# gaspachoo/EEG2Video

Measured on AMD Instinct MI355X. Metric: 6-frame 288x512 clips/sec (50-step DDIM), higher is better.
Workload: dtype f32; 1 GPU; 1xMI355X: batch=8/GPU synthetic latents [B,4,6,36,64] + [B,77,768] cond, 50-step DDIM, CFG 12.5, 288x512x6 VAE decode, fp32 (BASELINE configs[1]); clips_per_gpu=8, ddim_steps=50, unet_samples_per_ddim_step=16, weights=random-init SD-v1-4 architecture, counter RNG seed 42/43, collective=none

## Files before the change

eeg2video_amd/csrc/attn.hip:

```cpp
#include "h16.h"
#include "kernels.h"
#include "prof.h"
#include "runtime.h"
#include "act_io.h"

#include <cstdlib>
#include <type_traits>

namespace e2v {

typedef float f32x16 __attribute__((ext_vector_type(16)));
typedef float f32x4 __attribute__((ext_vector_type(4)));

struct AttnBlock { int qb, head, sf; bool valid; };
__host__ __device__ __forceinline__ int attn_xcd_unit(const int n, const int F, const int heads) {
    return n % 8 == 0 ? 0 : (n * F) % 8 == 0 ? 1 : 2;
}
__device__ __forceinline__ AttnBlock attn_block_of(const AttnArgs& p, const int nqb) {
    const int b = blockIdx.x, xcd = b & 7, idx = b >> 3;
    const int S = p.n * p.F;
    const int unit = attn_xcd_unit(p.n, p.F, p.heads);
    AttnBlock r;
    if (unit == 0) {
        const int per = p.F * p.heads * nqb;
        const int ul = idx / per, w = idx - ul * per;
        const int smp = ul * 8 + xcd;
        const int f = w / (p.heads * nqb), w2 = w - f * (p.heads * nqb);
        r.sf = smp * p.F + f; r.head = w2 / nqb; r.qb = w2 - r.head * nqb; r.valid = smp < p.n;
    } else if (unit == 1) {
        const int per = p.heads * nqb;
        const int ul = idx / per, w = idx - ul * per;
        r.sf = ul * 8 + xcd; r.head = w / nqb; r.qb = w - r.head * nqb; r.valid = r.sf < S;
    } else {
        const int ul = idx / nqb;
        const int pair = ul * 8 + xcd;
        r.qb = idx - ul * nqb; r.sf = pair / p.heads; r.head = pair - r.sf * p.heads; r.valid = pair < S * p.heads;
    }
    return r;
}
__device__ __forceinline__ AttnBlock attn_block(const AttnArgs& p) { return attn_block_of(p, (p.Nq + 127) / 128); }
static inline unsigned attn_grid_of(const AttnArgs& a, const unsigned nqb) {
    const int unit = attn_xcd_unit(a.n, a.F, a.heads);
    if (unit == 0) return 8u * (a.n / 8) * (unsigned)(a.F * a.heads) * nqb;
    if (unit == 1) return 8u * ((a.n * a.F) / 8) * (unsigned)a.heads * nqb;
    return 8u * ((a.n * a.F * a.heads + 7) / 8) * nqb;
}
static inline unsigned attn_grid(const AttnArgs& a) { return attn_grid_of(a, (a.Nq + 127) / 128); }

std::string attn_shape_tag(const AttnArgs& a) {
    return " D" + std::to_string(a.D) + " Nq" + std::to_string(a.Nq) + " Nk" + std::to_string(a.Nk) + " n" + std::to_string(a.n) + " F" + std::to_string(a.F) +
           " h" + std::to_string(a.heads);
}

template <int D>
__global__ __launch_bounds__(256) void flash_attn_kernel(const AttnArgs p) {
    constexpr int LD = D + 4;
    constexpr int TF = D / 32;
    constexpr bool VREM = (D - 32 * TF) == 8;
    constexpr int T = VREM ? TF : (D + 31) / 32;
    constexpr int TA = T > 0 ? T : 1;
    constexpr int G = D / 8;
    constexpr int DQ = D / 4;
    constexpr int KT = 32;
    constexpr int NF4 = KT * DQ;
    constexpr int LPT = (NF4 + 255) / 256;
    extern __shared__ __attribute__((aligned(16))) float smem[];

    const int tid = threadIdx.x;
    const int lane = tid & 63, wave = tid >> 6;
    const int j = lane & 31, h = lane >> 5;
    const AttnBlock blk = attn_block(p);
    if (!blk.valid) return;
    const int sf = blk.sf;
    const int smp = sf / p.F, f = sf - smp * p.F;
    const int head = blk.head;
    const int q0 = (blk.qb * 4 + wave) * 32;
    const bool active = q0 < p.Nq;

    int nseg = 1;
    size_t kvbase[2];
    if (p.mode == 0) {
        kvbase[0] = (size_t)(smp * p.F) * p.Nk;
        kvbase[1] = (size_t)(smp * p.F + (f > 0 ? f - 1 : 0)) * p.Nk;
        nseg = f >= 2 ? 2 : 1;
    } else {
        kvbase[0] = kvbase[1] = (size_t)smp * p.Nk;
    }
    const int tps = (p.Nk + KT - 1) / KT;
    const int ntiles = nseg * tps;

    f32x4 qf[G];
    {
        const int qrow = min(q0 + j, p.Nq - 1);
        const float* qp = p.q + ((size_t)sf * p.Nq + qrow) * p.ldq + head * D + h * 4;
        const float c = p.scale * 1.44269504088896340736f;
#pragma unroll
        for (int g = 0; g < G; ++g) {
            qf[g] = *reinterpret_cast<const f32x4*>(qp + g * 8);
            qf[g] *= c;
        }
    }

    constexpr unsigned OOB = 0x80000000u;
    auto rsrc_of = [](const void* ptr) {
        const unsigned long long v = reinterpret_cast<unsigned long long>(ptr);
        const unsigned lo = __builtin_amdgcn_readfirstlane((unsigned)v);
        const unsigned hi = __builtin_amdgcn_readfirstlane((unsigned)(v >> 32));
        return __builtin_amdgcn_make_buffer_rsrc(reinterpret_cast<void*>(((unsigned long long)hi << 32) | lo), (short)0, 0x7FFFFFF0,
                                                 0x00020000);
    };
    int ld_row[LPT];
    unsigned ld_off[LPT];
#pragma unroll
    for (int e = 0; e < LPT; ++e) {
        const int idx = tid + 256 * e;
        const int row = idx / DQ, c4 = idx - row * DQ;
        ld_row[e] = row;
        ld_off[e] = idx < NF4 ? (unsigned)(row * p.ldkv + c4 * 4) * 4u : OOB;
    }
    f32x4 kreg[LPT], vreg[LPT];
    auto load_tile = [&](int tt) {
        const int seg = tt / tps;
        const int key0 = (tt - seg * tps) * KT;
        const size_t first = (kvbase[seg] + key0) * p.ldkv + head * D;
        const __amdgpu_buffer_rsrc_t rk = rsrc_of(p.k + first), rv = rsrc_of(p.v + first);
        const int left = p.Nk - key0;
#pragma unroll
        for (int e = 0; e < LPT; ++e) {
            unsigned off = ld_off[e];
            if (left < KT) off = ld_row[e] < left ? off : OOB;
            kreg[e] = __builtin_bit_cast(f32x4, __builtin_amdgcn_raw_buffer_load_b128(rk, off, 0, 0));
            vreg[e] = __builtin_bit_cast(f32x4, __builtin_amdgcn_raw_buffer_load_b128(rv, off, 0, 0));
        }
    };
    auto store_tile = [&](int buf) {
        float* Ks = smem + buf * (2 * KT * LD);
        float* Vs = Ks + KT * LD;
#pragma unroll
        for (int e = 0; e < LPT; ++e) {
            const int idx = tid + 256 * e;
            if (idx < NF4) {
                const int row = idx / DQ, c4 = idx - row * DQ;
                *reinterpret_cast<f32x4*>(Ks + row * LD + c4 * 4) = kreg[e];
                *reinterpret_cast<f32x4*>(Vs + row * LD + c4 * 4) = vreg[e];
            }
        }
    };

    f32x16 acc[TA];
#pragma unroll
    for (int t = 0; t < TA; ++t)
#pragma unroll
        for (int r = 0; r < 16; ++r) acc[t][r] = 0.f;
    f32x4 rem0 = {0.f, 0.f, 0.f, 0.f}, rem1 = {0.f, 0.f, 0.f, 0.f};
    float m_i = -INFINITY, l_i = 0.f;

    load_tile(0);
    store_tile(0);
    __syncthreads();

    for (int tt = 0; tt < ntiles; ++tt) {
        const int buf = tt & 1;
        if (tt + 1 < ntiles) load_tile(tt + 1);
        const int seg_c = tt / tps;
        const int kbase = (tt - seg_c * tps) * KT;
        auto tile_body = [&](const int key0, const int sub, auto ragged) {
            const float* Ks = smem + buf * (2 * KT * LD) + sub * 32 * LD;
            const float* Vs = smem + buf * (2 * KT * LD) + KT * LD + sub * 32 * LD;
            const f32x16 zero16 = {0.f, 0.f, 0.f, 0.f, 0.f, 0.f, 0.f, 0.f, 0.f, 0.f, 0.f, 0.f, 0.f, 0.f, 0.f, 0.f};
            f32x16 st;
            const float* kp = Ks + j * LD + h * 4;
#pragma unroll
            for (int g = 0; g < G; ++g) {
                const f32x4 kf = *reinterpret_cast<const f32x4*>(kp + g * 8);
#pragma unroll
                for (int s = 0; s < 4; ++s)
                    st = __builtin_amdgcn_mfma_f32_32x32x2f32(kf[s], qf[g][s], (g == 0 && s == 0) ? zero16 : st, 0, 0, 0);
            }
            if constexpr (decltype(ragged)::value) {
#pragma unroll
                for (int r = 0; r < 16; ++r) {
                    const int key = key0 + (r & 3) + 8 * (r >> 2) + 4 * h;
                    if (key >= p.Nk) st[r] = -INFINITY;
                }
            }
            float mt = st[0];
#pragma unroll
            for (int r = 1; r < 16; ++r) mt = __builtin_fmaxf(mt, st[r]);
            mt = __builtin_fmaxf(mt, __shfl_xor(mt, 32));
            const float m_new = __builtin_fmaxf(m_i, mt);
            const bool moved = __any(m_new > m_i);
            float ps = 0.f;
#pragma unroll
            for (int r = 0; r < 16; ++r) {
                st[r] = __builtin_amdgcn_exp2f(st[r] - m_new);
                ps += st[r];
            }
            float alpha = 1.0f;
            if (moved) {
                alpha = __builtin_amdgcn_exp2f(m_i - m_new);
                l_i *= alpha;
            }
            l_i += ps;
            m_i = m_new;
#pragma unroll
            for (int t = 0; t < T; ++t) {
                if (moved) {
#pragma unroll
                    for (int r = 0; r < 16; ++r) acc[t][r] *= alpha;
                }
                const int dv = min(t * 32 + j, D - 1);
                const float* vp = Vs + (4 * h) * LD + dv;
#pragma unroll
                for (int r = 0; r < 16; ++r) {
                    const float vv = vp[((r & 3) + 8 * (r >> 2)) * LD];
                    acc[t] = __builtin_amdgcn_mfma_f32_32x32x2f32(vv, st[r], acc[t], 0, 0, 0);
                }
            }
            if constexpr (VREM) {
                if (moved) {
                    rem0 *= alpha;
                    rem1 *= alpha;
                }
                const float* vr = Vs + (4 * h) * LD + 32 * TF;
#pragma unroll
                for (int r = 0; r < 16; ++r) {
                    const float* row = vr + ((r & 3) + 8 * (r >> 2)) * LD;
                    const f32x4 v0 = *reinterpret_cast<const f32x4*>(row);
                    const f32x4 v1 = *reinterpret_cast<const f32x4*>(row + 4);
                    rem0 += v0 * st[r];
                    rem1 += v1 * st[r];
                }
            }
        };
#pragma unroll
        for (int sub = 0; sub < KT / 32; ++sub) {
            const int key0 = kbase + 32 * sub;
            if (active && key0 < p.Nk) {
                if (key0 + 32 <= p.Nk) tile_body(key0, sub, std::false_type{});
                else tile_body(key0, sub, std::true_type{});
            }
        }
        if (tt + 1 < ntiles) store_tile(buf ^ 1);
        __syncthreads();
    }

    const float l_tot = l_i + __shfl_xor(l_i, 32);
    if constexpr (VREM) {
#pragma unroll
        for (int e = 0; e < 4; ++e) {
            rem0[e] += __shfl_xor(rem0[e], 32);
            rem1[e] += __shfl_xor(rem1[e], 32);
        }
    }
    if (active && q0 + j < p.Nq) {
        const float inv = 1.0f / l_tot;
        float* op = p.o + ((size_t)sf * p.Nq + q0 + j) * p.ldo + head * D;
#pragma unroll
        for (int t = 0; t < T; ++t)
#pragma unroll
            for (int rg = 0; rg < 4; ++rg) {
                const int dv = t * 32 + 8 * rg + 4 * h;
                if (dv < D) {
                    f32x4 o;
#pragma unroll
                    for (int e = 0; e < 4; ++e) o[e] = acc[t][rg * 4 + e] * inv;
                    *reinterpret_cast<f32x4*>(op + dv) = o;
                }
            }
        if constexpr (VREM) {
            const f32x4 o = (h ? rem1 : rem0) * inv;
            *reinterpret_cast<f32x4*>(op + 32 * TF + 4 * h) = o;
        }
    }
}

typedef __bf16 abf16x4 __attribute__((ext_vector_type(4)));
typedef __bf16 abf16x8 __attribute__((ext_vector_type(8)));

template <typename H, int D, bool FOLD, int KT>
__global__ __launch_bounds__(256) void flash_attn_b16io_kernel(const AttnArgs p) {
    constexpr int DP = (D + 15) / 16 * 16;
    constexpr int KS = DP / 16;
    constexpr int T = (D + 31) / 32;
    constexpr int KROW = DP * 2 + 16;
    constexpr int VROW = ((T * 16) % 32 == 16) ? T * 64 : T * 64 + 64;
    constexpr int KBYTES = KT * KROW, VBYTES = KT * VROW;
    constexpr int STAGE = (KBYTES + VBYTES + 15) / 16 * 16;
    constexpr bool SUMV = (D % 32) != 0;
    constexpr int LROW = D % 32, LREG = 4 * (LROW / 8) + (LROW & 3), LHALF = (LROW >> 2) & 1;
    constexpr int C8 = D / 8;
    constexpr int NP = KT * C8;
    constexpr int LPT = (NP + 255) / 256;
    extern __shared__ __attribute__((aligned(16))) char smem_h[];

    const int tid = threadIdx.x;
    const int lane = tid & 63, wave = tid >> 6;
    const int j = lane & 31, h = lane >> 5;
    const AttnBlock blk = attn_block(p);
    if (!blk.valid) return;
    const int sf = blk.sf;
    const int smp = sf / p.F, f = sf - smp * p.F;
    const int head = blk.head;
    const int q0 = (blk.qb * 4 + wave) * 32;
    const bool active = q0 < p.Nq;
    const H* __restrict__ Q = reinterpret_cast<const H*>(p.q);
    const H* __restrict__ K = reinterpret_cast<const H*>(p.k);
    const H* __restrict__ V = reinterpret_cast<const H*>(p.v);

    int nseg = 1;
    size_t kvbase[2];
    if (p.mode == 0) {
        kvbase[0] = (size_t)(smp * p.F) * p.Nk;
        kvbase[1] = (size_t)(smp * p.F + (f > 0 ? f - 1 : 0)) * p.Nk;
        nseg = f >= 2 ? 2 : 1;
    } else {
        kvbase[0] = kvbase[1] = (size_t)smp * p.Nk;
    }
    const int tps = (p.Nk + KT - 1) / KT;
    const int ntiles = nseg * tps;

    for (int i = tid * 16; i < 2 * STAGE; i += 256 * 16)
        *reinterpret_cast<f32x4*>(smem_h + i) = f32x4{0.f, 0.f, 0.f, 0.f};
    if constexpr (SUMV) {
        __syncthreads();
        if (tid < 2 * KT)
            *reinterpret_cast<H*>(smem_h + (tid / KT) * STAGE + KBYTES + (tid % KT) * VROW + D * 2) = (H)1.0f;
    }

    hx8<H> qf[KS];
    {
        const int qrow = min(q0 + j, p.Nq - 1);
        const H* qp = Q + ((size_t)sf * p.Nq + qrow) * p.ldq + head * D;
#pragma unroll
        for (int s = 0; s < KS; ++s) {
            const int k0 = 16 * s + 8 * h;
            hx8<H> a;
#pragma unroll
            for (int e = 0; e < 8; ++e) a[e] = (H)0.f;
            if (k0 < D) a = *reinterpret_cast<const hx8<H>*>(qp + k0);
            if constexpr (FOLD) {
                const float qs = p.scale * 1.44269504088896340736f;
#pragma unroll
                for (int e = 0; e < 8; ++e) a[e] = (H)((float)a[e] * qs);
            }
            qf[s] = a;
        }
    }
    const float sc = p.scale * 1.44269504088896340736f;
    __syncthreads();

    constexpr unsigned OOB = 0x80000000u;
    auto rsrc_of = [](const void* ptr) {
        const unsigned long long v = reinterpret_cast<unsigned long long>(ptr);
        const unsigned lo = __builtin_amdgcn_readfirstlane((unsigned)v);
        const unsigned hi = __builtin_amdgcn_readfirstlane((unsigned)(v >> 32));
        return __builtin_amdgcn_make_buffer_rsrc(reinterpret_cast<void*>(((unsigned long long)hi << 32) | lo), (short)0, 0x7FFFFFF0,
                                                 0x00020000);
    };
    int ld_row[LPT], ld_c8[LPT];
    unsigned ld_off[LPT];
#pragma unroll
    for (int e = 0; e < LPT; ++e) {
        const int idx = tid + 256 * e;
        const int row = idx / C8, c8 = idx - row * C8;
        ld_row[e] = row; ld_c8[e] = c8;
        ld_off[e] = idx < NP ? (unsigned)(row * p.ldkv + c8 * 8) * 2u : OOB;
    }
    f32x4 kreg[LPT], vreg[LPT];
    auto load_tile = [&](const int seg, const int key0) {
        const size_t first = (kvbase[seg] + key0) * p.ldkv + head * D;
        const __amdgpu_buffer_rsrc_t rk = rsrc_of(K + first), rv = rsrc_of(V + first);
        const int left = p.Nk - key0;
#pragma unroll
        for (int e = 0; e < LPT; ++e) {
            unsigned off = ld_off[e];
            if (left < KT) off = ld_row[e] < left ? off : OOB;
            kreg[e] = __builtin_bit_cast(f32x4, __builtin_amdgcn_raw_buffer_load_b128(rk, off, 0, 0));
            vreg[e] = __builtin_bit_cast(f32x4, __builtin_amdgcn_raw_buffer_load_b128(rv, off, 0, 0));
        }
    };
    auto store_tile = [&](int buf) {
        char* Kl = smem_h + buf * STAGE;
        char* Vl = Kl + KBYTES;
#pragma unroll
        for (int e = 0; e < LPT; ++e) {
            if (tid + 256 * e < NP) {
                *reinterpret_cast<f32x4*>(Kl + ld_row[e] * KROW + ld_c8[e] * 16) = kreg[e];
                *reinterpret_cast<f32x4*>(Vl + ld_row[e] * VROW + ld_c8[e] * 16) = vreg[e];
            }
        }
    };

    f32x16 acc[T];
#pragma unroll
    for (int t = 0; t < T; ++t)
#pragma unroll
        for (int r = 0; r < 16; ++r) acc[t][r] = 0.f;
    float m_i = -INFINITY, l_i = 0.f;
    f32x16 negm;
#pragma unroll
    for (int r = 0; r < 16; ++r) negm[r] = 0.f;

    load_tile(0, 0);
    store_tile(0);
    __syncthreads();

    const int ti = lane & 15;
    const int tr_off = (4 * h + (ti >> 2)) * VROW + (16 * ((lane >> 4) & 1) + 4 * (ti & 3)) * 2;

    int key0 = 0;
    for (int tt = 0; tt < ntiles; ++tt) {
        const int buf = tt & 1;
        if (tt == tps) key0 = 0;
        if (tt + 1 < ntiles) {
            if (tt + 1 == tps) load_tile(1, 0); else load_tile(tt + 1 > tps ? 1 : 0, key0 + KT);
        }
#pragma unroll
        for (int sub = 0; sub < KT / 32; ++sub) {
        const int keyb = key0 + 32 * sub;
        if (active && keyb < p.Nk) {
            const char* Kl = smem_h + buf * STAGE + sub * 32 * KROW;
            const char* Vl = smem_h + buf * STAGE + KBYTES + sub * 32 * VROW;
            const f32x16 zero16 = {0.f, 0.f, 0.f, 0.f, 0.f, 0.f, 0.f, 0.f, 0.f, 0.f, 0.f, 0.f, 0.f, 0.f, 0.f, 0.f};
            f32x16 st;
            const char* kp = Kl + j * KROW + h * 16;
#pragma unroll
            for (int s = 0; s < KS; ++s) {
// ... 465 lines not shown
                for (int x = 0; x < 4; ++x) {
                    unsigned v1, v2, v3;
                    split3(vreg[e][x], v1, v2, v3);
                    char* vd = Vl + (c4 * 4 + x) * VROW + row * 2;
                    *reinterpret_cast<unsigned short*>(vd) = (unsigned short)(v1 >> 16);
                    *reinterpret_cast<unsigned short*>(vd + VBYTES) = (unsigned short)(v2 >> 16);
                    *reinterpret_cast<unsigned short*>(vd + 2 * VBYTES) = (unsigned short)(v3 >> 16);
                }
            }
        }
    };

    f32x16 acc[T];
#pragma unroll
    for (int t = 0; t < T; ++t)
#pragma unroll
        for (int r = 0; r < 16; ++r) acc[t][r] = 0.f;
    float m_i = -INFINITY, l_i = 0.f;

    load_tile(0);
    store_tile(0);
    __syncthreads();

    constexpr int TA[6] = {1, 2, 0, 1, 0, 0}, TB[6] = {1, 0, 2, 0, 1, 0};
    for (int tt = 0; tt < ntiles; ++tt) {
        const int buf = tt & 1;
        if (tt + 1 < ntiles) load_tile(tt + 1);
        const int seg_c = tt / tps;
        const int key0 = (tt - seg_c * tps) * 32;
        if (active) {
            const char* Kl = smem_x + buf * STAGE;
            const char* Vl = Kl + 3 * KBYTES;
            f32x16 st;
#pragma unroll
            for (int r = 0; r < 16; ++r) st[r] = 0.f;
            const char* kp = Kl + j * KROW + h * 16;
#pragma unroll
            for (int s = 0; s < KS; ++s) {
                abf16x8 kf[3];
#pragma unroll
                for (int pl = 0; pl < 3; ++pl) kf[pl] = *reinterpret_cast<const abf16x8*>(kp + pl * KBYTES + s * 32);
#pragma unroll
                for (int t6 = 0; t6 < 6; ++t6)
                    st = __builtin_amdgcn_mfma_f32_32x32x16_bf16(kf[TA[t6]], __builtin_bit_cast(abf16x8, qf[TB[t6]][s]), st, 0, 0, 0);
            }
            if (key0 + 32 > p.Nk) {
#pragma unroll
                for (int r = 0; r < 16; ++r) {
                    const int key = key0 + (r & 3) + 8 * (r >> 2) + 4 * h;
                    if (key >= p.Nk) st[r] = -INFINITY;
                }
            }
            float mt = st[0];
#pragma unroll
            for (int r = 1; r < 16; ++r) mt = __builtin_fmaxf(mt, st[r]);
            mt = __builtin_fmaxf(mt, __shfl_xor(mt, 32));
            const float m_new = __builtin_fmaxf(m_i, mt);
            const bool moved = __any(m_new > m_i);
            float ps = 0.f;
#pragma unroll
            for (int r = 0; r < 16; ++r) {
                st[r] = __builtin_amdgcn_exp2f(st[r] - m_new);
                ps += st[r];
            }
            float alpha = 1.0f;
            if (moved) {
                alpha = __builtin_amdgcn_exp2f(m_i - m_new);
                l_i *= alpha;
            }
            l_i += ps;
            m_i = m_new;
            au32x4 pf[3][2];
#pragma unroll
            for (int s = 0; s < 2; ++s)
#pragma unroll
                for (int e = 0; e < 4; ++e) {
                    unsigned a1, a2, a3, b1, b2, b3;
                    split3(st[8 * s + 2 * e], a1, a2, a3);
                    split3(st[8 * s + 2 * e + 1], b1, b2, b3);
                    pf[0][s][e] = (a1 >> 16) | (b1 & 0xFFFF0000u);
                    pf[1][s][e] = (a2 >> 16) | (b2 & 0xFFFF0000u);
                    pf[2][s][e] = (a3 >> 16) | (b3 & 0xFFFF0000u);
                }
#pragma unroll
            for (int t = 0; t < T; ++t) {
                if (moved) {
#pragma unroll
                    for (int r = 0; r < 16; ++r) acc[t][r] *= alpha;
                }
                const char* vrow = Vl + min(t * 32 + j, D - 1) * VROW + h * 8;
#pragma unroll
                for (int s = 0; s < 2; ++s) {
                    abf16x8 vf[3];
#pragma unroll
                    for (int pl = 0; pl < 3; ++pl) {
                        const abf16x4 lo = *reinterpret_cast<const abf16x4*>(vrow + pl * VBYTES + s * 32);
                        const abf16x4 hi = *reinterpret_cast<const abf16x4*>(vrow + pl * VBYTES + s * 32 + 16);
                        vf[pl] = __builtin_shufflevector(lo, hi, 0, 1, 2, 3, 4, 5, 6, 7);
                    }
#pragma unroll
                    for (int t6 = 0; t6 < 6; ++t6)
                        acc[t] = __builtin_amdgcn_mfma_f32_32x32x16_bf16(vf[TA[t6]], __builtin_bit_cast(abf16x8, pf[TB[t6]][s]), acc[t], 0, 0, 0);
                }
            }
        }
        if (tt + 1 < ntiles) store_tile(buf ^ 1);
        __syncthreads();
    }

    const float l_tot = l_i + __shfl_xor(l_i, 32);
    if (active && q0 + j < p.Nq) {
        const float inv = 1.0f / l_tot;
        float* op = p.o + ((size_t)sf * p.Nq + q0 + j) * p.ldo + head * D;
#pragma unroll
        for (int t = 0; t < T; ++t)
#pragma unroll
            for (int rg = 0; rg < 4; ++rg) {
                const int dv = t * 32 + 8 * rg + 4 * h;
                if (dv < D) {
                    f32x4 o;
#pragma unroll
                    for (int e = 0; e < 4; ++e) o[e] = acc[t][rg * 4 + e] * inv;
                    *reinterpret_cast<f32x4*>(op + dv) = o;
                }
            }
    }
}
template <int D>
static void launch_flash_x3(const AttnArgs& a, hipStream_t s) {
    constexpr int DP = (D + 15) / 16 * 16;
    constexpr size_t stage = ((size_t)3 * (32 * (DP * 2 + 16) + ((D + 31) / 32) * 32 * 72) + 15) / 16 * 16;
    constexpr size_t smem = 2 * stage;
    E2V_KATTR(&flash_attn_x3_kernel<D>, smem);
    dim3 grid(attn_grid(a), 1, 1);
    const double nk = a.mode == 0 ? 2.0 * a.Nk : (double)a.Nk;
    const double probs = (double)a.n * a.F * a.heads;
    ProfScope ps(a.mode == 0 ? "flash_attn_f32x3_sparse_causal" : "flash_attn_f32x3_cross", 4.0 * probs * a.Nq * nk * D,
                 4.0 * probs * D * (2.0 * a.Nq + 2.0 * (a.mode == 0 ? a.Nk : (double)a.Nk / a.F)), s);
    E2V_KLAUNCH((flash_attn_x3_kernel<D>), grid, dim3(256), smem, s, a);
}

template <int D>
static void launch_flash(const AttnArgs& a, hipStream_t s) {
    constexpr size_t smem = (size_t)2 * 2 * 32 * (D + 4) * sizeof(float);
    E2V_KATTR(&flash_attn_kernel<D>, smem);
    dim3 grid(attn_grid(a), 1, 1);
    const double nk = a.mode == 0 ? 2.0 * a.Nk : (double)a.Nk;
    const double probs = (double)a.n * a.F * a.heads;
    std::string pname = a.mode == 0 ? "flash_attn_sparse_causal" : "flash_attn_cross";
    if (prof_detail()) pname += attn_shape_tag(a);
    ProfScope ps(pname.c_str(), 4.0 * probs * a.Nq * nk * D,
                 4.0 * probs * D * (2.0 * a.Nq + 2.0 * (a.mode == 0 ? a.Nk : (double)a.Nk / a.F)), s);
    dry_tag(" -> flash_attn_kernel");
    E2V_KLAUNCH((flash_attn_kernel<D>), grid, dim3(256), smem, s, a);
}

bool flash_attention_supports(int D) {
    switch (D) {
        case 8: case 16: case 32: case 40: case 64: case 80: case 160: return true;
        default: return false;
    }
}

void flash_attention(const AttnArgs& a, hipStream_t s) {
    if (!flash_attention_supports(a.D))
        throw Error(E2V_EINVAL, "attention head dim " + std::to_string(a.D) + " has no kernel instance (supported: 8, 16, 32, 40, 64, 80, 160)");
    if (a.io_bf16) {
        if ((a.ldq | a.ldkv | a.ldo) & 7) throw Error(E2V_ESHAPE, "bf16 attention: row strides must be multiples of 8 elements");
        switch (a.D) {
            case 8: launch_flash_b16io<8>(a, s); return;
            case 16: launch_flash_b16io<16>(a, s); return;
            case 32: launch_flash_b16io<32>(a, s); return;
            case 40: launch_flash_b16io<40>(a, s); return;
            case 64: launch_flash_b16io<64>(a, s); return;
            case 80: launch_flash_b16io<80>(a, s); return;
            default: launch_flash_b16io<160>(a, s); return;
        }
    }
    if (a.x3) {
        switch (a.D) {
            case 8: launch_flash_x3<8>(a, s); return;
            case 16: launch_flash_x3<16>(a, s); return;
            case 32: launch_flash_x3<32>(a, s); return;
            case 40: launch_flash_x3<40>(a, s); return;
            case 64: launch_flash_x3<64>(a, s); return;
            case 80: launch_flash_x3<80>(a, s); return;
            default: launch_flash_x3<160>(a, s); return;
        }
    }
    switch (a.D) {
        case 8: launch_flash<8>(a, s); break;
        case 16: launch_flash<16>(a, s); break;
        case 32: launch_flash<32>(a, s); break;
        case 40: launch_flash<40>(a, s); break;
        case 64: launch_flash<64>(a, s); break;
        case 80: launch_flash<80>(a, s); break;
        default: launch_flash<160>(a, s); break;
    }
}

static constexpr int FMAX = 8;
template <typename T>
__global__ __launch_bounds__(256) void temporal_attn_kernel(const T* __restrict__ qkv, int ld, T* __restrict__ out,
                                                            int ldo, int n, int F, int HW, int heads, int D, float scale) {
    const size_t total = (size_t)n * HW * heads * F;
    const size_t gid = blockIdx.x * (size_t)blockDim.x + threadIdx.x;
    if (gid >= total) return;
    const int i = gid % F;
    const int head = (gid / F) % heads;
    const size_t ph = gid / ((size_t)F * heads);
    const int pix = ph % HW;
    const int smp = ph / HW;
    const int C = heads * D;
    const size_t row0 = (size_t)smp * F * HW + pix;
    const T* qp = qkv + (row0 + (size_t)i * HW) * ld + head * D;
    const T* kp = qkv + row0 * ld + C + head * D;
    const T* vp = qkv + row0 * ld + 2 * C + head * D;
    const size_t fstride = (size_t)HW * ld;
    float s[FMAX];
#pragma unroll
    for (int jf = 0; jf < FMAX; ++jf) s[jf] = 0.f;
    for (int c = 0; c < D; c += 4) {
        const f32x4 qv = ld4(qp + c);
#pragma unroll
        for (int jf = 0; jf < FMAX; ++jf)
            if (jf < F) {
                const f32x4 kv = ld4(kp + jf * fstride + c);
                s[jf] += qv[0] * kv[0] + qv[1] * kv[1] + qv[2] * kv[2] + qv[3] * kv[3];
            }
    }
    float m = -INFINITY;
#pragma unroll
    for (int jf = 0; jf < FMAX; ++jf)
        if (jf < F) {
            s[jf] *= scale;
            m = fmaxf(m, s[jf]);
        }
    float l = 0.f;
#pragma unroll
    for (int jf = 0; jf < FMAX; ++jf)
        if (jf < F) {
            s[jf] = expf(s[jf] - m);
            l += s[jf];
        }
    const float inv = 1.0f / l;
    T* op = out + (row0 + (size_t)i * HW) * ldo + head * D;
    for (int c = 0; c < D; c += 4) {
        f32x4 o = {0.f, 0.f, 0.f, 0.f};
#pragma unroll
        for (int jf = 0; jf < FMAX; ++jf)
            if (jf < F) {
                const f32x4 vv = ld4(vp + jf * fstride + c);
                o += vv * (s[jf] * inv);
            }
        st4(op + c, o);
    }
}

template <typename T>
__global__ __launch_bounds__(128) void temporal_attn_lds_kernel(const T* __restrict__ qkv, int ld, T* __restrict__ out,
                                                                int ldo, int F, int HW, int C, int D, float scale, int PB,
                                                                int CS, int npg) {
    extern __shared__ __attribute__((aligned(16))) float sm[];
    const int smp = blockIdx.x / npg, p0 = (blockIdx.x - smp * npg) * PB;
    const int c_base = blockIdx.y * CS;
    if constexpr (!std::is_same<T, float>::value) {
        const int CO = CS / 8;
        const int total = F * PB * 3 * CO;
        for (int idx = threadIdx.x; idx < total; idx += 128) {
            const int c8 = idx % CO;
            int r = idx / CO;
            const int part = r % 3; r /= 3;
            const int pp = r % PB;
            const int f = r / PB;
            const int pix = p0 + pp;
            f32x4 lo = {0.f, 0.f, 0.f, 0.f}, hi = lo;
            if (pix < HW) {
                const hx8<T> v = *reinterpret_cast<const hx8<T>*>(qkv + ((size_t)(smp * F + f) * HW + pix) * ld + part * C + c_base + c8 * 8);
#pragma unroll
                for (int e = 0; e < 4; ++e) { lo[e] = (float)v[e]; hi[e] = (float)v[4 + e]; }
            }
            *reinterpret_cast<f32x4*>(sm + (size_t)idx * 8) = lo;
            *reinterpret_cast<f32x4*>(sm + (size_t)idx * 8 + 4) = hi;
        }
    } else {
        const int CQ = CS / 4;
        const int total = F * PB * 3 * CQ;
        for (int idx = threadIdx.x; idx < total; idx += 128) {
            const int c4 = idx % CQ;
            int r = idx / CQ;
            const int part = r % 3; r /= 3;
            const int pp = r % PB;
            const int f = r / PB;
            const int pix = p0 + pp;
            f32x4 v = {0.f, 0.f, 0.f, 0.f};
            if (pix < HW) v = ld4(qkv + ((size_t)(smp * F + f) * HW + pix) * ld + part * C + c_base + c4 * 4);
            *reinterpret_cast<f32x4*>(sm + (size_t)idx * 4) = v;
        }
    }
    __syncthreads();
    const int hs = CS / D;
    const int items = PB * hs * F;
    for (int item = threadIdx.x; item < items; item += 128) {
        const int i = item % F;
        const int hh = (item / F) % hs;
        const int pp = item / (F * hs);
// ... 495 lines not shown
```

eeg2video_amd/csrc/bgemm.hip:

```cpp
#include "igemm_epi.h"
#include "prof.h"
#include "runtime.h"

#include <cstdio>
#include <cstdlib>
#include <string>

#include <map>
#include <mutex>

namespace e2v {

static std::mutex& knob_mutex() { static std::mutex m; return m; }
static std::map<std::string, int>& knob_table() { static std::map<std::string, int> t; return t; }
int* knob(const char* name, int dflt) {
    std::lock_guard<std::mutex> lk(knob_mutex());
    auto& t = knob_table();
    auto it = t.find(name);
    if (it == t.end()) {
        const char* e = std::getenv(name);
        it = t.emplace(name, e ? std::atoi(e) : dflt).first;
    }
    return &it->second;
}
bool set_knob(const char* name, int value) {
    std::lock_guard<std::mutex> lk(knob_mutex());
    auto& t = knob_table();
    auto it = t.find(name);
    if (it == t.end()) {
        static const char* const known[] = {"E2V_BGEMM_PERS", "E2V_BGEMM_256LIN", "E2V_BGEMM_256", "E2V_BGEMM_T256", "E2V_BGEMM_T256P", "E2V_BGEMM_T256P_BIAS_LDS",
                                            "E2V_ATTN_KT64", "E2V_ATTN_Q64", "E2V_ATTN_CROSS_RESIDENT", "E2V_TATTN_WAVE", "E2V_LN_ROWS", "E2V_BGEMM_UP2X",
                                            "E2V_SPLITK", "E2V_SPLITK_FORCE", "E2V_GN_FUSED_SMALL", "E2V_BGEMM_S3_SMALL", "E2V_SMALL_FAMILY_CLIPS", "E2V_POOL_GUARD",
                                            "E2V_OP_IO16", "E2V_OP_RECORD"
#ifdef E2V_AB
                                            , "E2V_BGEMM_S3", "E2V_BGEMM_LIN", "E2V_BGEMM_T256_TAIL", "E2V_ATTN_FOLD", "E2V_ATTN_Q64P", "E2V_ATTN_Q64_NW", "E2V_GN_ROWS", "E2V_GN_GROUP_MB", "E2V_GN_SKIP_PARTIAL", "E2V_GN_RB", "E2V_GN_RB_EPILOGUE",
                                            "E2V_BGEMM_256_MINROUNDS", "E2V_BGEMM_T256_MINK", "E2V_BGEMM_T256_MINTILES", "E2V_BGEMM_T256P_MAXK", "E2V_BGEMM_T256P_MINTILES", "E2V_GN_CHUNK_ROWS",
                                            "E2V_GN_CHUNK_ROWS_SMALL", "E2V_IGEMM_HALF_BELOW", "E2V_SPLITK_MIN_DEPTH", "E2V_SPLITK_MAX_TILES", "E2V_GN_COOP", "E2V_LN_STATS_ONLY"
#endif
#ifdef E2V_ABLATE
                                            , "E2V_BGEMM_ABLATE"
#endif
        };
        bool ok = false;
        for (const char* k : known) ok = ok || std::string(k) == name;
        if (!ok) return false;
        it = t.emplace(name, value).first;
    }
    it->second = value;
    return true;
}

int pool_guard_kib() {
    static const int* const kib = knob("E2V_POOL_GUARD", 0);
    return *kib > 0 ? *kib : 0;
}

template <class F, int... T>
__device__ __forceinline__ void static_for_taps(F&& f, std::integer_sequence<int, T...>) {
    (f(std::integral_constant<int, T>{}), ...);
}

template <typename H, int BM, int BN, int WGM, int WGN, int STAGE = 128 * 128 * 2, bool LIN = false, int NST = 2, int CALLER = 0>
__device__ __forceinline__ void bgemm_tile(const IgemmArgs& p, const int rbg, const int n0, char* smem) {
    constexpr int BKE = 64;
    constexpr int ROWB = 128;
    constexpr int NW = WGM * WGN, NT = 64 * NW;
    constexpr int WM = BM / WGM, WN = BN / WGN;
    constexpr int TM = WM / 32, TN = WN / 32;
    constexpr int A_BYTES = BM * ROWB, B_BYTES = BN * ROWB;
    constexpr int APW = BM / 8 / NW, BPW = BN / 8 / NW;
    static_assert(APW >= 1 && BPW >= 1 && A_BYTES + B_BYTES <= STAGE, "tile does not fit the stage");
    const int z = p.batch > 1 ? rbg / p.nbm_per : 0;
    const int bm = rbg - z * p.nbm_per;

    const int tid = threadIdx.x;
    const int lane = tid & 63;
    const int wave = __builtin_amdgcn_readfirstlane(tid >> 6);
    const int wm = wave / WGN, wn = wave % WGN;

    const H* __restrict__ a0 = reinterpret_cast<const H*>(p.a0) + (size_t)z * p.sa0;
    const H* __restrict__ a1 = reinterpret_cast<const H*>(p.a1);
    const char* __restrict__ w = reinterpret_cast<const char*>(p.w16) + ((size_t)z * p.sw + (size_t)n0 * p.ldw) * 2;

    const int steps0 = (p.c0 + BKE - 1) / BKE, steps1 = (p.c1 + BKE - 1) / BKE;
    const int nk = p.taps * (steps0 + steps1);

    unsigned* tab = reinterpret_cast<unsigned*>(smem + NST * STAGE);
    const int hw_out = p.Ho * p.Wo, hw_in = p.Hs * p.Ws;
    const int img0 = p.taps == 1 ? 0 : (bm * BM) / hw_out;
    const size_t row_base = p.taps == 1 ? (size_t)bm * BM : (size_t)img0 * hw_in;
    for (int e = tid; !LIN && e < p.taps * BM; e += NT) {
        const int tap = e / BM, row = e - tap * BM;
        const int m = bm * BM + row;
        unsigned pix = ~0u;
        if (m < p.M) {
            if (p.taps == 1) {
                pix = (unsigned)row;
            } else {
                const int img = m / hw_out;
                const int rem = m - img * hw_out;
                const int oy = rem / p.Wo, ox = rem - oy * p.Wo;
                const int ky = (tap * 11) >> 5, kx = tap - 3 * ky;
                const int iy = oy * p.stride - p.pad + ky, ix = ox * p.stride - p.pad + kx;
                if ((unsigned)iy < (unsigned)p.Hi && (unsigned)ix < (unsigned)p.Wi) {
                    int sy = iy, sx = ix;
                    if (p.upsample) {
                        sy = min((int)floorf((float)iy * p.ups_h), p.Hs - 1);
                        sx = min((int)floorf((float)ix * p.ups_w), p.Ws - 1);
                    }
                    pix = (unsigned)(((img - img0) * p.Hs + sy) * p.Ws + sx);
                }
            }
        }
        tab[e] = pix;
    }
    constexpr unsigned OOB = 0x80000000u;
    const H* const a0b = a0 + row_base * p.lda0;
    const H* const a1b = p.c1 > 0 ? a1 + row_base * p.lda1 : a0b;
    const int a_records = (p.ablate & 2) ? 0 : 0x7FFFFFF0;
    auto rsrc_of = [](const void* ptr, const int records = 0x7FFFFFF0) {
        const unsigned long long v = reinterpret_cast<unsigned long long>(ptr);
        const unsigned lo = __builtin_amdgcn_readfirstlane((unsigned)v);
        const unsigned hi = __builtin_amdgcn_readfirstlane((unsigned)(v >> 32));
        return __builtin_amdgcn_make_buffer_rsrc(reinterpret_cast<void*>(((unsigned long long)hi << 32) | lo), (short)0, records,
                                                 0x00020000);
    };
    const __amdgpu_buffer_rsrc_t rw = rsrc_of(w);

    const int r8 = lane >> 3, pp = lane & 7;
    int a_row[APW];
    unsigned a_kc[APW];
#pragma unroll
    for (int i = 0; i < APW; ++i) {
        a_row[i] = 8 * (wave * APW + i) + r8;
        a_kc[i] = (unsigned)(pp ^ ((a_row[i] >> 1) & 7));
    }
    unsigned b_off[BPW], b_kc[BPW];
#pragma unroll
    for (int j = 0; j < BPW; ++j) {
        const int r = 8 * (wave * BPW + j) + r8;
        b_kc[j] = (unsigned)(pp ^ ((r >> 1) & 7));
        b_off[j] = (n0 + r < p.N) ? (unsigned)(r * p.ldw * 2) + b_kc[j] * 16u : OOB;
    }
    unsigned a_voff0[APW], a_voff1[APW];
#pragma unroll
    for (int i = 0; i < APW; ++i) {
        const bool in = bm * BM + a_row[i] < p.M;
        a_voff0[i] = in ? (unsigned)(a_row[i] * p.lda0 * 2) + a_kc[i] * 16u : OOB;
        a_voff1[i] = in ? (unsigned)(a_row[i] * p.lda1 * 2) + a_kc[i] * 16u : OOB;
    }
    if constexpr (!LIN) __syncthreads();

    int k_src = 0, k_cb = 0, k_tap = 0, cseg = p.c0, ldb = p.lda0 * 2;
    bool done = false;
    unsigned pixn[APW];
    if constexpr (!LIN) {
#pragma unroll
        for (int i = 0; i < APW; ++i) pixn[i] = tab[a_row[i]];
    }
    typedef __attribute__((address_space(3))) void* lds_ptr;
    auto issue = [&](const int buf) {
        char* Ab = smem + buf * STAGE;
        char* Bb = Ab + A_BYTES;
        if constexpr (LIN) {
            if (!done) {
                const unsigned so = (unsigned)k_cb * 2u;
                const unsigned sob = (unsigned)((k_src ? p.c0 : 0) + k_cb) * 2u;
                const bool whole = k_cb + BKE <= cseg;
                const __amdgpu_buffer_rsrc_t rsa = rsrc_of(k_src ? a1b : a0b, a_records);
#pragma unroll
                for (int i = 0; i < APW; ++i) {
                    const unsigned vo = k_src ? a_voff1[i] : a_voff0[i];
                    const unsigned off = (whole || k_cb + (int)a_kc[i] * 8 < cseg) ? vo : OOB;
                    __builtin_amdgcn_raw_ptr_buffer_load_lds(rsa, (lds_ptr)(Ab + (wave * APW + i) * 1024), 16, off, so, 0, 0);
                }
#pragma unroll
                for (int j = 0; j < BPW; ++j) {
                    const unsigned off = (whole || k_cb + (int)b_kc[j] * 8 < cseg) ? b_off[j] : OOB;
                    __builtin_amdgcn_raw_ptr_buffer_load_lds(rw, (lds_ptr)(Bb + (wave * BPW + j) * 1024), 16, off, sob, 0, 0);
                }
                k_cb += BKE;
                if (k_cb >= cseg) {
                    if (k_src == 0 && p.c1 > 0) { k_src = 1; k_cb = 0; cseg = p.c1; }
                    else done = true;
                }
            }
            return;
        }
// ... 899 lines not shown
```

Before: 0.5929 clips/s.

## Add lean f32 flash-attention kernel with buffer loads and register-staged double buffering

Replaces the default f32 flash-attention kernel with a leaner variant. K/V tiles are prefetched into registers through raw buffer loads with out-of-bounds clamping and stored to double-buffered LDS after compute, so loads overlap the MFMA work. Cross-half reductions use v_permlane32_swap, the accumulator rescale is skipped when no lane's max grows, and LDS offsets are precomputed. The old kernel stays available under an A/B knob, at the cost of more register pressure and reliance on gfx950-specific instructions.

```diff
diff --git a/eeg2video_amd/csrc/attn.hip b/eeg2video_amd/csrc/attn.hip
--- a/eeg2video_amd/csrc/attn.hip
+++ b/eeg2video_amd/csrc/attn.hip
@@ -52,8 +52,9 @@
            " h" + std::to_string(a.heads);
 }
 
+#ifdef E2V_AB
 template <int D>
-__global__ __launch_bounds__(256) void flash_attn_kernel(const AttnArgs p) {
+__device__ __forceinline__ void flash_attn_f32_plain(const AttnArgs& p) {
     constexpr int LD = D + 4;
     constexpr int TF = D / 32;
     constexpr bool VREM = (D - 32 * TF) == 8;
@@ -274,6 +275,267 @@
         }
     }
 }
+#endif
+
+__device__ __forceinline__ void xhalf_pair(const float x, float& a, float& b) {
+    a = x; b = x;
+    asm volatile("s_nop 1\n\tv_permlane32_swap_b32 %0, %1" : "+v"(a), "+v"(b));
+}
+
+template <int D>
+__device__ __forceinline__ void flash_attn_f32_lean(const AttnArgs& p) {
+    constexpr int LD = D + 4;
+    constexpr int TF = D / 32;
+    constexpr bool VREM = (D - 32 * TF) == 8;
+    constexpr int T = VREM ? TF : (D + 31) / 32;
+    constexpr int TA = T > 0 ? T : 1;
+    constexpr int G = D / 8;
+    constexpr int DQ = D / 4;
+    constexpr int KT = 32;
+    constexpr int NF4 = KT * DQ;
+    constexpr int LPT = (NF4 + 255) / 256;
+    extern __shared__ __attribute__((aligned(16))) float smem[];
+
+    const int tid = threadIdx.x;
+    const int lane = tid & 63, wave = tid >> 6;
+    const int j = lane & 31, h = lane >> 5;
+    const AttnBlock blk = attn_block(p);
+    if (!blk.valid) return;
+    const int sf = blk.sf;
+    const int smp = sf / p.F, f = sf - smp * p.F;
+    const int head = blk.head;
+    const int q0 = (blk.qb * 4 + wave) * 32;
+    const int qleft = p.Nq - __builtin_amdgcn_readfirstlane(q0);
+
+    int nseg = 1;
+    size_t kvbase0, kvbase1;
+    if (p.mode == 0) {
+        kvbase0 = (size_t)(smp * p.F) * p.Nk;
+        kvbase1 = (size_t)(smp * p.F + (f > 0 ? f - 1 : 0)) * p.Nk;
+        nseg = f >= 2 ? 2 : 1;
+    } else {
+        kvbase0 = kvbase1 = (size_t)smp * p.Nk;
+    }
+    const int tps = (p.Nk + KT - 1) / KT;
+    const int ntiles = nseg * tps;
+
+    f32x4 qf[G];
+    {
+        const int qrow = min(q0 + j, p.Nq - 1);
+        const float* qp = p.q + ((size_t)sf * p.Nq + qrow) * p.ldq + head * D + h * 4;
+        const float c = p.scale * 1.44269504088896340736f;
+#pragma unroll
+        for (int g = 0; g < G; ++g) {
+            qf[g] = *reinterpret_cast<const f32x4*>(qp + g * 8);
+            qf[g] *= c;
+        }
+    }
+
+    constexpr unsigned OOB = 0x80000000u;
+    auto rsrc_of = [](const void* ptr, const int bytes) {
+        const unsigned long long v = reinterpret_cast<unsigned long long>(ptr);
+        const unsigned lo = __builtin_amdgcn_readfirstlane((unsigned)v);
+        const unsigned hi = __builtin_amdgcn_readfirstlane((unsigned)(v >> 32));
+        return __builtin_amdgcn_make_buffer_rsrc(reinterpret_cast<void*>(((unsigned long long)hi << 32) | lo), (short)0, bytes, 0x00020000);
+    };
+    unsigned ld_off[LPT];
+#pragma unroll
+    for (int e = 0; e < LPT; ++e) {
+        const int idx = tid + 256 * e;
+        const int row = idx / DQ, c4 = idx - row * DQ;
+        ld_off[e] = idx < NF4 ? (unsigned)(row * p.ldkv + c4 * 4) * 4u : OOB;
+    }
+    f32x4 kreg[LPT], vreg[LPT];
+    auto load_tile = [&](const int seg, const int key0) {
+        const size_t first = ((seg ? kvbase1 : kvbase0) + key0) * p.ldkv + head * D;
+        const int keys = min(p.Nk - key0, KT);
+        const int bytes = keys * p.ldkv * 4;
+        const __amdgpu_buffer_rsrc_t rk = rsrc_of(p.k + first, bytes), rv = rsrc_of(p.v + first, bytes);
+#pragma unroll
+        for (int e = 0; e < LPT; ++e) {
+            kreg[e] = __builtin_bit_cast(f32x4, __builtin_amdgcn_raw_buffer_load_b128(rk, ld_off[e], 0, 0));
+            vreg[e] = __builtin_bit_cast(f32x4, __builtin_amdgcn_raw_buffer_load_b128(rv, ld_off[e], 0, 0));
+        }
+    };
+    auto store_tile = [&](const int buf) {
+        float* Ks = smem + buf * (2 * KT * LD);
+        float* Vs = Ks + KT * LD;
+#pragma unroll
+        for (int e = 0; e < LPT; ++e) {
+            const int idx = tid + 256 * e;
+            if (idx < NF4) {
+                const int row = idx / DQ, c4 = idx - row * DQ;
+                *reinterpret_cast<f32x4*>(Ks + row * LD + c4 * 4) = kreg[e];
+                *reinterpret_cast<f32x4*>(Vs + row * LD + c4 * 4) = vreg[e];
+            }
+        }
+    };
+
+    constexpr bool VPIN = 3 * LD + 32 * (TA - 1) <= 255;
+    unsigned kb_off[2], vb_off[2][4];
+#pragma unroll
+    for (int b = 0; b < 2; ++b) {
+        kb_off[b] = (unsigned)(b * (2 * KT * LD) + j * LD + h * 4) * 4u;
+        asm volatile("" : "+v"(kb_off[b]));
+#pragma unroll
+        for (int g = 0; g < 4; ++g) {
+            vb_off[b][g] = (unsigned)(b * (2 * KT * LD) + KT * LD + (8 * g + 4 * h) * LD + min(j, D - 1)) * 4u;
+            if constexpr (VPIN) asm volatile("" : "+v"(vb_off[b][g]));
+        }
+    }
+    const char* const smem_b = reinterpret_cast<const char*>(smem);
+
+    f32x16 acc[TA];
+#pragma unroll
+    for (int t = 0; t < TA; ++t)
+#pragma unroll
+        for (int r = 0; r < 16; ++r) acc[t][r] = 0.f;
+    f32x4 rem0 = {0.f, 0.f, 0.f, 0.f}, rem1 = {0.f, 0.f, 0.f, 0.f};
+    float m_i = -INFINITY, l_i = 0.f;
+
+    auto tile_body = [&](auto bufc, const int key0) {
+        constexpr int buf = decltype(bufc)::value;
+        const float* Vs = smem + buf * (2 * KT * LD) + KT * LD;
+        const f32x16 zero16 = {0.f, 0.f, 0.f, 0.f, 0.f, 0.f, 0.f, 0.f, 0.f, 0.f, 0.f, 0.f, 0.f, 0.f, 0.f, 0.f};
+        f32x16 st;
+        const float* kp = reinterpret_cast<const float*>(smem_b + kb_off[buf]);
+#pragma unroll
+        for (int g = 0; g < G; ++g) {
+            const f32x4 kf = *reinterpret_cast<const f32x4*>(kp + g * 8);
+#pragma unroll
+            for (int s = 0; s < 4; ++s)
+                st = __builtin_amdgcn_mfma_f32_32x32x2f32(kf[s], qf[g][s], (g == 0 && s == 0) ? zero16 : st, 0, 0, 0);
+        }
+        if (key0 + 32 > p.Nk) {
+            asm volatile("" ::: "memory");
+#pragma unroll
+            for (int r = 0; r < 16; ++r) {
+                const int key = key0 + (r & 3) + 8 * (r >> 2) + 4 * h;
+                if (key >= p.Nk) st[r] = -INFINITY;
+            }
+        }
+        float mt = st[0];
+#pragma unroll
+        for (int r = 1; r < 16; ++r) mt = __builtin_fmaxf(mt, st[r]);
+        {
+            float a, b;
+            xhalf_pair(mt, a, b);
+            mt = __builtin_fmaxf(a, b);
+        }
+        const float m_new = __builtin_fmaxf(m_i, mt);
+        if (__any(m_new > m_i)) {
+            asm volatile("" ::: "memory");
+            const float alpha = __builtin_amdgcn_exp2f(m_i - m_new);
+            l_i *= alpha;
+#pragma unroll
+            for (int t = 0; t < T; ++t)
+#pragma unroll
+                for (int r = 0; r < 16; ++r) acc[t][r] *= alpha;
+            if constexpr (VREM) {
+                rem0 *= alpha;
+                rem1 *= alpha;
+            }
+        }
+        float ps = 0.f;
+#pragma unroll
+        for (int r = 0; r < 16; ++r) {
+            st[r] = __builtin_amdgcn_exp2f(st[r] - m_new);
+            ps += st[r];
+        }
+        l_i += ps;
+        m_i = m_new;
+#pragma unroll
+        for (int t = 0; t < T; ++t) {
+            const int dt = min(t * 32 + j, D - 1) - min(j, D - 1);
+#pragma unroll
+            for (int r = 0; r < 16; ++r) {
+                const float vv = reinterpret_cast<const float*>(smem_b + vb_off[buf][r >> 2])[(r & 3) * LD + dt];
+                acc[t] = __builtin_amdgcn_mfma_f32_32x32x2f32(vv, st[r], acc[t], 0, 0, 0);
+            }
+        }
+        if constexpr (VREM) {
+            const float* vr = Vs + (4 * h) * LD + 32 * TF;
+#pragma unroll
+            for (int r = 0; r < 16; ++r) {
+                const float* row = vr + ((r & 3) + 8 * (r >> 2)) * LD;
+                const f32x4 v0 = *reinterpret_cast<const f32x4*>(row);
+                const f32x4 v1 = *reinterpret_cast<const f32x4*>(row + 4);
+                rem0 += v0 * st[r];
+                rem1 += v1 * st[r];
+            }
+        }
+    };
+
+    load_tile(0, 0);
+    store_tile(0);
+    __syncthreads();
+
+    int tt = 0;
+    int lseg = 0, lkey = 0;
+    auto step = [&](auto bufc) {
+        constexpr int buf = decltype(bufc)::value;
+        const int key0 = lkey;
+        int more = ntiles - 1 - tt;
+        asm volatile("" : "+s"(more));
+        if (more > 0) {
+            lkey += KT;
+            if (lkey >= p.Nk) { lkey = 0; lseg = 1; }
+            load_tile(lseg, lkey);
+        }
+        int work = qleft;
+        asm volatile("" : "+s"(work));
+        if (work > 0) tile_body(bufc, key0);
+        if (more > 0) store_tile(buf ^ 1);
+        __syncthreads();
+    };
+    for (;;) {
+        step(std::integral_constant<int, 0>{});
+        if (++tt >= ntiles) break;
+        step(std::integral_constant<int, 1>{});
+        if (++tt >= ntiles) break;
+    }
+
+    auto xhalf_sum = [](const float x) {
+        float a, b;
+        xhalf_pair(x, a, b);
+        return a + b;
+    };
+    const float l_tot = xhalf_sum(l_i);
+    if constexpr (VREM) {
+#pragma unroll
+        for (int e = 0; e < 4; ++e) {
+            rem0[e] = xhalf_sum(rem0[e]);
+            rem1[e] = xhalf_sum(rem1[e]);
+        }
+    }
+    if (q0 + j < p.Nq) {
+        const float inv = 1.0f / l_tot;
+        float* op = p.o + ((size_t)sf * p.Nq + q0 + j) * p.ldo + head * D;
+#pragma unroll
+        for (int t = 0; t < T; ++t)
+#pragma unroll
+            for (int rg = 0; rg < 4; ++rg) {
+                const int dv = t * 32 + 8 * rg + 4 * h;
+                if (dv < D) {
+                    f32x4 o;
+#pragma unroll
+                    for (int e = 0; e < 4; ++e) o[e] = acc[t][rg * 4 + e] * inv;
+                    *reinterpret_cast<f32x4*>(op + dv) = o;
+                }
+            }
+        if constexpr (VREM) {
+            const f32x4 o = (h ? rem1 : rem0) * inv;
+            *reinterpret_cast<f32x4*>(op + 32 * TF + 4 * h) = o;
+        }
+    }
+}
+
+template <int D>
+__global__ __launch_bounds__(256) void flash_attn_kernel(const AttnArgs p) { flash_attn_f32_lean<D>(p); }
+#ifdef E2V_AB
+template <int D>
+__global__ __launch_bounds__(256) void flash_attn_plain_kernel(const AttnArgs p) { flash_attn_f32_plain<D>(p); }
+#endif
 
 typedef __bf16 abf16x4 __attribute__((ext_vector_type(4)));
 typedef __bf16 abf16x8 __attribute__((ext_vector_type(8)));
@@ -1045,6 +1307,14 @@
     ProfScope ps(pname.c_str(), 4.0 * probs * a.Nq * nk * D,
                  4.0 * probs * D * (2.0 * a.Nq + 2.0 * (a.mode == 0 ? a.Nk : (double)a.Nk / a.F)), s);
     dry_tag(" -> flash_attn_kernel");
+#ifdef E2V_AB
+    static const int* const lean = E2V_AB_KNOB("E2V_ATTN_F32_LEAN", 1);
+    if (!*lean) {
+        E2V_KATTR(&flash_attn_plain_kernel<D>, smem);
+        E2V_KLAUNCH((flash_attn_plain_kernel<D>), grid, dim3(256), smem, s, a);
+        return;
+    }
+#endif
     E2V_KLAUNCH((flash_attn_kernel<D>), grid, dim3(256), smem, s, a);
 }
 
diff --git a/eeg2video_amd/csrc/bgemm.hip b/eeg2video_amd/csrc/bgemm.hip
--- a/eeg2video_amd/csrc/bgemm.hip
+++ b/eeg2video_amd/csrc/bgemm.hip
@@ -33,7 +33,7 @@
                                             "E2V_SPLITK", "E2V_SPLITK_FORCE", "E2V_GN_FUSED_SMALL", "E2V_BGEMM_S3_SMALL", "E2V_SMALL_FAMILY_CLIPS", "E2V_POOL_GUARD",
                                             "E2V_OP_IO16", "E2V_OP_RECORD"
 #ifdef E2V_AB
-                                            , "E2V_BGEMM_S3", "E2V_BGEMM_LIN", "E2V_BGEMM_T256_TAIL", "E2V_ATTN_FOLD", "E2V_ATTN_Q64P", "E2V_ATTN_Q64_NW", "E2V_GN_ROWS", "E2V_GN_GROUP_MB", "E2V_GN_SKIP_PARTIAL", "E2V_GN_RB", "E2V_GN_RB_EPILOGUE",
+                                            , "E2V_BGEMM_S3", "E2V_BGEMM_LIN", "E2V_BGEMM_T256_TAIL", "E2V_ATTN_FOLD", "E2V_ATTN_F32_LEAN", "E2V_ATTN_Q64P", "E2V_ATTN_Q64_NW", "E2V_GN_ROWS", "E2V_GN_GROUP_MB", "E2V_GN_SKIP_PARTIAL", "E2V_GN_RB", "E2V_GN_RB_EPILOGUE",
                                             "E2V_BGEMM_256_MINROUNDS", "E2V_BGEMM_T256_MINK", "E2V_BGEMM_T256_MINTILES", "E2V_BGEMM_T256P_MAXK", "E2V_BGEMM_T256P_MINTILES", "E2V_GN_CHUNK_ROWS",
                                             "E2V_GN_CHUNK_ROWS_SMALL", "E2V_IGEMM_HALF_BELOW", "E2V_SPLITK_MIN_DEPTH", "E2V_SPLITK_MAX_TILES", "E2V_GN_COOP", "E2V_LN_STATS_ONLY"
 #endif
```

Result: no change. 0.5983 clips/s, median of 6 (+0.9%).
